# ShinYwings/SingleHDR-tf2

Measured on AMD Instinct MI355X. Metric: HDR images/sec (512x512) end-to-end inference, deq+lin+hal, higher is better.
Workload: dtype f32

## Files before the change

include/shdr.h:

```cpp
#ifndef SHDR_H_
#define SHDR_H_

#include <stdint.h>

#ifdef __cplusplus
extern "C" {
#endif

void shdr_config_reload(void);

#define SHDR_OK          0
#define SHDR_E_SHAPE    (-1)
#define SHDR_E_ALIGN    (-2)
#define SHDR_E_ARCH     (-3)
#define SHDR_E_LAUNCH   (-4)
#define SHDR_E_NULL     (-5)

#define SHDR_ACT_NONE   0
#define SHDR_ACT_RELU   1
#define SHDR_ACT_LRELU  2
#define SHDR_ACT_TANH   3

#define SHDR_ALGO_AUTO    0
#define SHDR_ALGO_MFMA    1
// ... 117 lines not shown
int shdr_invcrf_decode_fwd_f32(const float* feat, const float* wfc, const float* bfc,
                               const float* table, float* out, int B, int F, int K,
                               void* stream);
int shdr_increase_fwd_f32(const float* rf, float* out, int B, int K, void* stream);
int shdr_apply_rf_fwd_f32(const float* x, const float* rf, float* y, int B,
                          int64_t n_per_batch, int K, void* stream);

int shdr_clip_fwd_f32(const float* x, float* y, int64_t n, float lo, float hi, void* stream);
int shdr_vgg_preprocess_fwd_f32(const float* x, float* y, int64_t npix, int out_channels,
                                void* stream);
int shdr_reverse3_fwd_f32(const float* x, float* y, int64_t npix, void* stream);
int shdr_alpha_blend_fwd_f32(const float* b, const float* hal, float* a, float* alpha_out,
                             int64_t npix, float thr, void* stream);
int shdr_pack3_fwd_f32(const float* s0, const float* s1, const float* s2, const float* s3,
                       int nsrc, float* y, int out_channels, int64_t npix, void* stream);
int shdr_pad_channels_f32(const float* x, float* y, int64_t npix, int Cin, int Cout, void* stream);
int shdr_logc_fwd_f32(const float* x, float* y, int64_t n, void* stream);
int shdr_affine_act_f32(const float* x, const float* scale, const float* shift, const float* residual, float* y,
                        int64_t npix, int C, int act, void* stream);

int shdr_act_bwd_f32(const float* dy, const float* y, float* dx, int64_t n, int act, void* stream);
int shdr_clip_bwd_f32(const float* dy, const float* x, float* dx, int64_t n, float lo, float hi, void* stream);
int shdr_add_f32(const float* a, const float* b, float* y, int64_t n, void* stream);
int shdr_add_ranged_f32(const float* a, const float* b, float* y, int64_t n, float* y_range, void* stream);
int shdr_avgpool2_bwd_f32(const float* dy, float* dx, int N, int H, int W, int C, void* stream);
int shdr_maxpool2_bwd_f32(const float* x, const float* dy, float* dx, int N, int H, int W, int C, void* stream);
int shdr_maxpool3s2_bwd_f32(const float* x, const float* y, const float* dy, float* dx, int N, int H, int W, int C, void* stream);
int shdr_resize2x_bwd_f32(const float* dy, float* dx, int N, int H, int W, int C, void* stream);
int shdr_resize2x_bwd_ranged_f32(const float* dy, float* dx, int N, int H, int W, int C, float* dx_range, void* stream);
int shdr_gap_bwd_f32(const float* dy, float* dx, int N, int HW, int C, void* stream);
// ... 346 lines not shown
```

singlehdr-tf2_amd/_lib.py:

```python
import ctypes
import os

_HERE = os.path.dirname(os.path.abspath(__file__))
LIB_PATH = os.environ.get("SHDR_LIB") or os.path.join(_HERE, "libshdr.so")

c_int = ctypes.c_int
c_i64 = ctypes.c_int64
c_f32 = ctypes.c_float
c_ptr = ctypes.c_void_p


class ConvDesc(ctypes.Structure):
    _fields_ = [("N", ctypes.c_int32), ("H", ctypes.c_int32), ("W", ctypes.c_int32),
                ("C1", ctypes.c_int32), ("C2", ctypes.c_int32),
                ("Cout", ctypes.c_int32), ("KH", ctypes.c_int32), ("KW", ctypes.c_int32),
                ("stride", ctypes.c_int32), ("pad_t", ctypes.c_int32), ("pad_l", ctypes.c_int32),
                ("Ho", ctypes.c_int32), ("Wo", ctypes.c_int32),
                ("x2_scale", ctypes.c_float),
                ("act1", ctypes.c_int32), ("act2", ctypes.c_int32),
                ("res_cstride", ctypes.c_int32), ("y_cstride", ctypes.c_int32),
                ("algo", ctypes.c_int32), ("cout_valid", ctypes.c_int32),
                ("w_batch_stride", ctypes.c_int64),
                ("y_pix_stride", ctypes.c_int32), ("y_off_h", ctypes.c_int32), ("y_off_w", ctypes.c_int32),
                ("y_H", ctypes.c_int32), ("y_W", ctypes.c_int32),
# ... 101 lines not shown
    "shdr_soft_hist_fwd_f32": (c_int, [c_ptr, c_ptr, c_i64, c_int, c_int, c_ptr]),
    "shdr_lin_frontend_fwd_f32": (c_int, [c_ptr, c_ptr, c_int, c_int, c_int, c_int, c_ptr]),
    "shdr_avgpool2_fwd_f32": (c_int, [c_ptr, c_ptr, c_int, c_int, c_int, c_int, c_ptr]),
    "shdr_maxpool2_fwd_f32": (c_int, [c_ptr, c_ptr, c_int, c_int, c_int, c_int, c_ptr]),
    "shdr_maxpool3s2_fwd_f32": (c_int, [c_ptr, c_ptr, c_int, c_int, c_int, c_int, c_ptr]),
    "shdr_resize2x_fwd_f32": (c_int, [c_ptr, c_ptr, c_int, c_int, c_int, c_int, c_ptr]),
    "shdr_gap_fwd_f32": (c_int, [c_ptr, c_ptr, c_int, c_int, c_int, c_ptr]),
    "shdr_invcrf_decode_fwd_f32": (c_int, [c_ptr] * 5 + [c_int, c_int, c_int, c_ptr]),
    "shdr_increase_fwd_f32": (c_int, [c_ptr, c_ptr, c_int, c_int, c_ptr]),
    "shdr_apply_rf_fwd_f32": (c_int, [c_ptr, c_ptr, c_ptr, c_int, c_i64, c_int, c_ptr]),
    "shdr_clip_fwd_f32": (c_int, [c_ptr, c_ptr, c_i64, c_f32, c_f32, c_ptr]),
    "shdr_vgg_preprocess_fwd_f32": (c_int, [c_ptr, c_ptr, c_i64, c_int, c_ptr]),
    "shdr_reverse3_fwd_f32": (c_int, [c_ptr, c_ptr, c_i64, c_ptr]),
    "shdr_alpha_blend_fwd_f32": (c_int, [c_ptr, c_ptr, c_ptr, c_ptr, c_i64, c_f32, c_ptr]),
    "shdr_pack3_fwd_f32": (c_int, [c_ptr] * 4 + [c_int, c_ptr, c_int, c_i64, c_ptr]),
    "shdr_logc_fwd_f32": (c_int, [c_ptr, c_ptr, c_i64, c_ptr]),
    "shdr_affine_act_f32": (c_int, [c_ptr] * 5 + [c_i64, c_int, c_int, c_ptr]),
    "shdr_pad_channels_f32": (c_int, [c_ptr, c_ptr, c_i64, c_int, c_int, c_ptr]),
    "shdr_act_bwd_f32": (c_int, [c_ptr, c_ptr, c_ptr, c_i64, c_int, c_ptr]),
    "shdr_clip_bwd_f32": (c_int, [c_ptr, c_ptr, c_ptr, c_i64, c_f32, c_f32, c_ptr]),
    "shdr_add_f32": (c_int, [c_ptr, c_ptr, c_ptr, c_i64, c_ptr]),
    "shdr_add_ranged_f32": (c_int, [c_ptr, c_ptr, c_ptr, c_i64, c_ptr, c_ptr]),
    "shdr_avgpool2_bwd_f32": (c_int, [c_ptr, c_ptr, c_int, c_int, c_int, c_int, c_ptr]),
    "shdr_maxpool2_bwd_f32": (c_int, [c_ptr, c_ptr, c_ptr, c_int, c_int, c_int, c_int, c_ptr]),
    "shdr_maxpool3s2_bwd_f32": (c_int, [c_ptr, c_ptr, c_ptr, c_ptr, c_int, c_int, c_int, c_int, c_ptr]),
    "shdr_resize2x_bwd_f32": (c_int, [c_ptr, c_ptr, c_int, c_int, c_int, c_int, c_ptr]),
    "shdr_resize2x_bwd_ranged_f32": (c_int, [c_ptr, c_ptr, c_int, c_int, c_int, c_int, c_ptr, c_ptr]),
    "shdr_gap_bwd_f32": (c_int, [c_ptr, c_ptr, c_int, c_int, c_int, c_ptr]),
    "shdr_upsample_zero2_f32": (c_int, [c_ptr, c_ptr, c_int, c_int, c_int, c_int, c_ptr]),
    "shdr_bn_stats_f32": (c_int, [c_ptr] * 6 + [c_i64, c_int, c_f32, c_ptr]),
# ... 99 lines not shown
```

singlehdr-tf2_amd/_ops.py:

```python
import collections
import ctypes
import math

import numpy as np
import torch

try:
    from . import _lib
except ImportError:
    import _lib

AUTOGRAD = None


def _needs_grad(*tensors):
    return AUTOGRAD is not None and torch.is_grad_enabled() and any(
        isinstance(t, torch.Tensor) and t.requires_grad for t in tensors)


WINOGRAD = True


ACT_NONE, ACT_RELU, ACT_LRELU, ACT_TANH = 0, 1, 2, 3
ALGO_AUTO, ALGO_MFMA, ALGO_DIRECT, ALGO_MFMA_REG = 0, 1, 2, 3
# ... 740 lines not shown
        return AUTOGRAD.pack3(list(srcs), out_channels, dtype)
    lib = _lib.load()
    srcs_in = list(srcs)
    srcs = [_pix3(s, "src%d" % i)[0] for i, s in enumerate(srcs)]
    n = len(srcs)
    if not 1 <= n <= 4:
        raise ValueError("pack3: 1..4 sources")
    if any(s.shape != srcs[0].shape for s in srcs):
        raise ValueError("pack3: shape mismatch")
    oc = out_channels or 3 * n
    y = torch.empty(tuple(srcs[0].shape[:-1]) + (oc,), device=srcs[0].device, dtype=dtype)
    p = [_ptr(s) for s in srcs] + [None] * (4 - n)
    if dtype == HALF:
        _lib.check(lib.shdr_pack3_f16(p[0], p[1], p[2], p[3], n, _ptr(y), oc, srcs[0].numel() // 3, 0, _stream()), "shdr_pack3_f16")
        return y
    _lib.check(lib.shdr_pack3_fwd_f32(p[0], p[1], p[2], p[3], n, _ptr(y), oc, srcs[0].numel() // 3,
                                      _stream()), "shdr_pack3_fwd_f32")
    if n == 1:
        return _carry_range(y, srcs_in[0])
    bounds = [_bound_of(t) for t in srcs_in]
    return y if None in bounds else set_bound(y, max(bounds))


def _conv_desc(x_shape, w_shape, stride, c2, x2_scale, cout_valid):
    n, h, wd, c1 = x_shape
    kh, kw, cin, cout_gemm = w_shape
    ho, pt = same_pad(h, kh, stride)
    wo, pl = same_pad(wd, kw, stride)
    d = _lib.ConvDesc()
    d.N, d.H, d.W, d.C1, d.C2 = n, h, wd, c1, c2
    d.Cout, d.KH, d.KW, d.stride = cout_gemm, kh, kw, stride
    d.cout_valid = cout_valid or cout_gemm
    d.pad_t, d.pad_l, d.Ho, d.Wo = pt, pl, ho, wo
    d.x2_scale = float(x2_scale)
    return d

# ... 1411 lines not shown
```

singlehdr-tf2_amd/build.py:

```python
import os
import shutil
import subprocess
import sys

HERE = os.path.dirname(os.path.abspath(__file__))
CSRC = os.path.join(HERE, "csrc")
INCLUDE = os.path.normpath(os.path.join(HERE, "..", "include"))
OBJ_DIR = os.path.join(HERE, "build")
LIB = os.path.join(HERE, "libshdr.so")

SOURCES = {
    "api.cpp": [],
    "conv.hip": [],
    "conv_plan.hip": [],
    "conv_x3.hip": [],
    "conv_x3n.hip": [],
    "conv_f16.hip": [],
    "conv_f16_patch.hip": [],
    "conv_f16_w3.hip": [],
    "wgrad_x3.hip": [],
    "wgrad_f16.hip": [],
    "wgrad_f16_alltaps.hip": [],
    "elem_f16.hip": ["-ffp-contract=off"],
    "wgrad.hip": [],
    "wgrad_winograd.hip": [],
    "bwd.hip": [],
    "finetune.hip": [],
    "winograd.hip": [],
    "winograd_fused.hip": [],
    "frontend.hip": ["-ffp-contract=off"],
    "pool.hip": [],
    "up2_lowres.hip": [],
    "up2_fused.hip": [],
    "crf.hip": [],
    "glue.hip": [],
    "imageio.hip": [],
    "hdr_rle.hip": [],
    "metrics.hip": [],
    "camera.hip": ["-ffp-contract=off"],
    "dataset.hip": ["-ffp-contract=off"],
    "exr.hip": ["-ffp-contract=off"],
    "exr_write.hip": ["-ffp-contract=off"],
    "deflate.hip": [],
    "deflate_lz.hip": [],
    "inflate.hip": [],
    "hdr_real.hip": ["-ffp-contract=off"],
    "jpeg.hip": ["-ffp-contract=off"],
    "jpeg_scan.hip": [],
}
COMMON = ["-O3", "-std=c++17", "-fPIC", "--offload-arch=gfx950", "-I" + INCLUDE, "-I" + CSRC,
# ... 8 lines not shown


def _stale(target, deps):
    if not os.path.exists(target):
        return True
    t = os.path.getmtime(target)
    return any(os.path.getmtime(d) > t for d in deps)


def build(force=False, verbose=True):
    hipcc = _hipcc()
    os.makedirs(OBJ_DIR, exist_ok=True)
    headers = [os.path.join(CSRC, "shdr_internal.h"), os.path.join(CSRC, "linear_resize.h"), os.path.join(CSRC, "jpeg_int.h"), os.path.join(CSRC, "deflate_huffman.h"),
               os.path.join(CSRC, "deflate_lz.h"), os.path.join(CSRC, "deflate_batch.h"),
               os.path.join(CSRC, "inflate.h"), os.path.join(CSRC, "jpeg_scan.h"),
               os.path.join(CSRC, "exr_half.h"), os.path.join(INCLUDE, "shdr.h"), __file__]
    objs = []
    procs = []
    for src, extra in SOURCES.items():
        s = os.path.join(CSRC, src)
        o = os.path.join(OBJ_DIR, os.path.splitext(src)[0] + ".o")
        objs.append(o)
        if force or _stale(o, [s] + headers):
            cmd = [hipcc] + COMMON + extra + ["-x", "hip", "-c", s, "-o", o]
            if verbose:
                print(" ".join(cmd), flush=True)
            procs.append((src, subprocess.Popen(cmd)))
    for src, p in procs:
        if p.wait() != 0:
            raise RuntimeError("hipcc failed on " + src)
    if force or procs or _stale(LIB, objs):
# ... 10 lines not shown
```

singlehdr-tf2_amd/csrc/up2_fused.hip:

```cpp
#include <hip/hip_fp16.h>
#include <stdlib.h>

#include <type_traits>

#include "shdr_internal.h"

namespace {

using f32x4 = __attribute__((ext_vector_type(4))) float;
using f16x8 = __attribute__((ext_vector_type(8))) _Float16;

inline hipStream_t S(void* s) { return reinterpret_cast<hipStream_t>(s); }

constexpr int UF_HEADER_FLOATS = 16;
constexpr int UF_IMG_HALVES = 64 * 32, UF_UNIT_HALVES = 2 * UF_IMG_HALVES;
constexpr int UF_R = 8;
constexpr int UF_COLS = 14;
constexpr int UF_MAX_CIN = 128;
constexpr int UF_THREADS = 256;
constexpr int uf_stride(int CMAX) { return CMAX == 32 ? 32 : CMAX + 8; }

struct UpFusedArgs {
  const float* x;
  const _Float16* wp;
  const float* hdr;
  const float* bias;
  const float* scale;
  const float* shift;
  const float* proj;
  float* y;
  float* yproj;
  const unsigned* xr;
  unsigned* yr;
  int N, h, w, C1, nty, ntx, act1, act2;
  int npatch;
};

__device__ __forceinline__ void uf_range_scale(const unsigned* r, float& xs, float& ixs) {
  xs = 1.0f;
  ixs = 1.0f;
  const unsigned b = r ? *r : 0u;
  if (b != 0u && b < 0x7f800000u) {
    int ex;
    frexpf(__uint_as_float(b), &ex);
    int T = 11 - ex;
    T = T < -126 ? -126 : (T > 126 ? 126 : T);
    xs = ldexpf(1.0f, T);
    ixs = ldexpf(1.0f, -T);
  }
}
// ... 35 lines not shown
  for (int e = 0; e < 4; ++e) r[e] = __int_as_float(__builtin_amdgcn_update_dpp(0, __float_as_int(a[e]), 0x111, 0xf, 0xf, true));
  return r;
}
__device__ __forceinline__ f32x4 from_right(f32x4 a) {
  f32x4 r;
#pragma unroll
  for (int e = 0; e < 4; ++e) r[e] = __int_as_float(__builtin_amdgcn_update_dpp(0, __float_as_int(a[e]), 0x101, 0xf, 0xf, true));
  return r;
}

__device__ __forceinline__ int uf_xcd_remap(int bid, int nwg) {
  const int q = nwg >> 3, r = nwg & 7, xcd = bid & 7, idx = bid >> 3;
  return (xcd < r ? xcd * (q + 1) : r * (q + 1) + (xcd - r) * q) + idx;
}

template <int R, int CW, int CMAX>
__global__ __launch_bounds__(UF_THREADS, 2) void up2_fused_kernel(const UpFusedArgs a) {
  constexpr int UF_STRIDE = uf_stride(CMAX);
  constexpr int COUT = 16 * CW, PPB = 4 / CW, GT = 64 * CW;
  constexpr int NPIX = 16 * R, IMG = NPIX * UF_STRIDE;
  constexpr int RO = R - 2;
  extern __shared__ __attribute__((aligned(16))) _Float16 fsm_all[];

  const int lane = threadIdx.x & 63;
  const int wave = __builtin_amdgcn_readfirstlane(threadIdx.x >> 6);
  const int ps = PPB == 1 ? 0 : wave / CW;
  const int cw = PPB == 1 ? wave : wave % CW;
  const int tid = PPB == 1 ? threadIdx.x : threadIdx.x & (GT - 1);
  _Float16* const fsm = fsm_all + ps * (2 * IMG);
  const float* const projp = CW == 4 ? a.proj : nullptr;
  int L = uf_xcd_remap(blockIdx.x, gridDim.x) * PPB + ps;
// ... 180 lines not shown
          ym = fmaxf(fmaxf(fmaxf(fmaxf(ym, fabsf(v[0])), fabsf(v[1])), fabsf(v[2])), fabsf(v[3]));
        }
        if (projp) {
#pragma unroll
          for (int j = 0; j < 3; ++j) {
            float t = v[0] * pq[j][0] + v[1] * pq[j][1] + v[2] * pq[j][2] + v[3] * pq[j][3];
            t += __shfl_xor(t, 16, 64);
            t += __shfl_xor(t, 32, 64);
            if (fg == 0) part[(cw * RO * 64 + (qo * 2 + r) * 32 + 2 * p + s) * 3 + j] = t;
          }
        }
      }
  }
  if (projp) {
    __syncthreads();
    for (int slot = tid; slot < RO * 64; slot += UF_THREADS) {
      const int s = slot & 1, pp = (slot >> 1) & 15, r = (slot >> 5) & 1, qo = slot >> 6;
      const int m0 = m_start + qo, jj = j_start - 1 + pp;
      if (m0 < a.h && pp >= 1 && pp <= UF_COLS && jj < a.w) {
        float* o = a.yproj + (((size_t)n * 2 * a.h + 2 * m0 + r) * 2 * a.w + 2 * jj + s) * 3;
#pragma unroll
        for (int j = 0; j < 3; ++j)
          o[j] = ((part[slot * 3 + j] + part[(RO * 64 + slot) * 3 + j]) + part[(2 * RO * 64 + slot) * 3 + j]) + part[(3 * RO * 64 + slot) * 3 + j];
      }
    }
  }
  if (a.y && a.yr) shdr::range_out_block256(a.yr, ym);
}

constexpr int uf_lds_bytes(int R, int CW, int CMAX) { return (4 / CW) * 2 * 16 * R * uf_stride(CMAX) * 2; }

bool uf_geometry_ok(const shdr_conv2d_desc* d) {
  return d && d->N > 0 && d->H > 0 && d->W > 0 && d->H % 2 == 0 && d->W % 2 == 0 && d->KH == 3 && d->KW == 3 && d->stride == 1 && d->pad_t == 1 &&
         d->pad_l == 1 && d->Ho == d->H && d->Wo == d->W && d->C2 == 0 && d->C1 % 32 == 0 && d->C1 <= UF_MAX_CIN;
}
bool uf_shape_ok(const shdr_conv2d_desc* d) { return uf_geometry_ok(d) && d->C1 >= 64 && d->Cout == 64; }
bool uf_narrow_shape_ok(const shdr_conv2d_desc* d) {
  return uf_geometry_ok(d) && d->C1 >= 32 && (d->Cout == 32 || (d->Cout == 16 && d->C1 <= 64));
// ... 5 lines not shown
  g->N = d->N; g->H = d->H / 2; g->W = d->W / 2; g->C1 = d->C1; g->C2 = 0;
  g->Cout = uf_narrow_columns(d->Cout);
  g->KH = 1; g->KW = 1; g->stride = 1; g->pad_t = 0; g->pad_l = 0; g->Ho = g->H; g->Wo = g->W;
  g->x2_scale = 1.0f; g->act1 = SHDR_ACT_NONE; g->act2 = SHDR_ACT_NONE; g->algo = SHDR_ALGO_AUTO; g->cout_valid = g->Cout; g->y_cstride = g->Cout;
  return true;
}
__global__ __launch_bounds__(256) void up2_fused_filter_kernel(const float* __restrict__ w, float* __restrict__ st, int Cin, int Cout, int Cp) {
  const long total = (long)Cin * Cp;
  for (long e = (long)blockIdx.x * 256 + threadIdx.x; e < total; e += (long)gridDim.x * 256) {
    const int col = (int)(e % Cp), ci = (int)(e / Cp);
    const int t = col / Cout, co = col - t * Cout;
    st[e] = t < 9 ? w[((size_t)t * Cin + ci) * Cout + co] : 0.0f;
  }
}

template <int CW, int CMAX>
int uf_launch(const UpFusedArgs& a, hipStream_t st) {
  constexpr int lds = uf_lds_bytes(UF_R, CW, CMAX), PPB = 4 / CW;
  static_assert(lds <= 160 * 1024 - 64, "the patch images of a block must fit the CU's LDS");
  static bool attr_done[shdr::kMaxDevices] = {};
  const int dev_slot = shdr::device_slot();
  if (!attr_done[dev_slot]) {
    hipError_t e = hipFuncSetAttribute(reinterpret_cast<const void*>(&up2_fused_kernel<UF_R, CW, CMAX>), hipFuncAttributeMaxDynamicSharedMemorySize, lds);
    if (e != hipSuccess) return shdr::fail(SHDR_E_ARCH, "hipFuncSetAttribute: %s", hipGetErrorString(e));
    attr_done[dev_slot] = true;
  }
  const long nblk = ((long)a.npatch + PPB - 1) / PPB;
  hipLaunchKernelGGL((up2_fused_kernel<UF_R, CW, CMAX>), dim3((unsigned)nblk), dim3(UF_THREADS), lds, st, a);
  return shdr::check_launch("up2_fused_kernel");
}

}

extern "C" int shdr_conv2d_up2_narrow_enabled(void) { return SHDR_ENV("SHDR_NO_UP2_NARROW") == nullptr ? 1 : 0; }

extern "C" int shdr_conv2d_up2_fused_ok_f32(const shdr_conv2d_desc* d) {
  const bool narrow = uf_narrow_shape_ok(d) && shdr_conv2d_up2_narrow_enabled();
  if (!(uf_shape_ok(d) || narrow) || SHDR_ENV("SHDR_NO_UP2_FUSED") != nullptr || SHDR_ENV("SHDR_NO_UP2_LOWRES") != nullptr ||
      SHDR_ENV("SHDR_NO_WINOGRAD") != nullptr || SHDR_ENV("SHDR_NO_X3") != nullptr)
    return 0;
  if (d->algo != SHDR_ALGO_AUTO || d->prologue != SHDR_PROLOGUE_BILINEAR2X) return 0;
  if ((d->cout_valid != 0 && d->cout_valid != d->Cout) || d->w_batch_stride != 0 || d->y_pix_stride > 1 || (d->y_cstride != 0 && d->y_cstride != d->Cout)) return 0;
  if (d->act1 == SHDR_ACT_TANH || d->act2 == SHDR_ACT_TANH) return 0;
// ... 11 lines not shown
extern "C" int shdr_conv2d_up2_fused_prepare_filter_f32(const shdr_conv2d_desc* d, const float* w, float* prepared, void* stream) {
  if (uf_shape_ok(d)) return shdr_conv2d_up2_lowres_prepare_filter_f32(d, w, prepared, stream);
  SHDR_REQUIRE(d && w && prepared, SHDR_E_NULL, "up2_fused_prepare_filter: null pointer");
  shdr_conv2d_desc g;
  SHDR_REQUIRE(uf_narrow_gemm_desc(d, &g), SHDR_E_SHAPE,
               "up2_fused_prepare_filter: need a 3x3 layer with one source, even H and W, and Cin 64 / 96 / 128 -> 64, Cin 32 .. 128 -> 32 or Cin 32 / 64 -> 16");
  const int64_t packed = shdr_conv2d_x3_filter_elems_f32(&g);
  SHDR_REQUIRE(packed > 0, SHDR_E_SHAPE, "up2_fused_prepare_filter: the 1x1 form of this layer has no packed filter");
  float* staged = prepared + packed;
  const long total = (long)g.C1 * g.Cout;
  hipLaunchKernelGGL(up2_fused_filter_kernel, dim3(shdr::stream_grid(total)), dim3(256), 0, S(stream), w, staged, g.C1, d->Cout, g.Cout);
  if (int rc = shdr::check_launch("up2_fused_filter")) return rc;
  return shdr_conv2d_x3_prepare_filter_f32(&g, staged, prepared, stream);
}

extern "C" int shdr_conv2d_fwd_up2_fused_f32(const shdr_conv2d_desc* d, const float* x, const float* prepared, const float* bias, const float* scale,
                                             const float* shift, const float* proj, float* y_proj, float* y, const float* x_range, float* y_range,
                                             void* stream) {
  SHDR_REQUIRE(d && x && prepared && x_range, SHDR_E_NULL, "conv2d_up2_fused: null desc / x / prepared filter / x_range");
  SHDR_REQUIRE(y || y_proj, SHDR_E_NULL, "conv2d_up2_fused: neither y nor y_proj");
  SHDR_REQUIRE((proj == nullptr) == (y_proj == nullptr), SHDR_E_NULL, "conv2d_up2_fused: proj and y_proj come together");
  SHDR_REQUIRE(shdr_conv2d_up2_fused_ok_f32(d), SHDR_E_SHAPE, "conv2d_up2_fused: layer not taken (shdr_conv2d_up2_fused_ok_f32)");
  SHDR_REQUIRE(!proj || d->Cout == 64, SHDR_E_SHAPE, "conv2d_up2_fused: the projected output is the 64-cout form's");
  SHDR_REQUIRE((scale == nullptr) == (shift == nullptr), SHDR_E_NULL, "conv2d_up2_fused: scale and shift come together");
  SHDR_REQUIRE(shdr::aligned16(x) && shdr::aligned16(prepared) && (!y || shdr::aligned16(y)) && (!bias || shdr::aligned16(bias)) &&
                   (!scale || (shdr::aligned16(scale) && shdr::aligned16(shift))) && (!proj || shdr::aligned16(proj)),
               SHDR_E_ALIGN, "conv2d_up2_fused: tensors must be 16-byte aligned");
  UpFusedArgs a{};
  a.x = x; a.hdr = prepared; a.wp = reinterpret_cast<const _Float16*>(prepared + UF_HEADER_FLOATS);
  a.bias = bias; a.scale = scale; a.shift = shift; a.proj = proj; a.y = y; a.yproj = y_proj;
  a.xr = reinterpret_cast<const unsigned*>(x_range); a.yr = reinterpret_cast<unsigned*>(y_range);
  a.N = d->N; a.h = d->H / 2; a.w = d->W / 2; a.C1 = d->C1; a.act1 = d->act1; a.act2 = d->act2;
  a.nty = (a.h + UF_R - 3) / (UF_R - 2);
  a.ntx = (a.w + UF_COLS - 1) / UF_COLS;
  a.npatch = (int)((long)a.N * a.nty * a.ntx);
  hipStream_t st = S(stream);
  if (d->Cout == 64) return uf_launch<4, 128>(a, st);
  if (d->Cout == 32) return d->C1 <= 64 ? uf_launch<2, 64>(a, st) : uf_launch<2, 128>(a, st);
  return d->C1 <= 32 ? uf_launch<1, 32>(a, st) : uf_launch<1, 64>(a, st);
}
```

singlehdr-tf2_amd/hallucination_net.py:

```python
import torch

try:
    from . import _ops as K
    from ._layers import Layer, Conv2D, BatchNormalization, is_training, taping
except ImportError:
    import _ops as K
    from _layers import Layer, Conv2D, BatchNormalization, is_training, taping


class down1(Layer):

    def __init__(self, inChannels, outChannels, device=None):
        super().__init__()
        self.conv1 = Conv2D(inChannels, outChannels, (3, 3), device=device)
        self.conv2 = Conv2D(outChannels, outChannels, (3, 3), device=device)

    def call(self, x, proj=None):
        if x.shape[-1] != self.conv1.kernel.shape[2]:
            x = self.conv1.call_padded(x, cin_pad=x.shape[-1], act1=K.ACT_RELU)
        else:
            x = self.conv1(x, act1=K.ACT_RELU)
        if proj is not None:
            r = K.conv2d_maxpool2(x, self.conv2.kernel, self.conv2.bias, act1=K.ACT_RELU, proj=proj)
            if r is not None:
# ... 27 lines not shown
        self.norm1 = BatchNormalization(outChannels, device=device)

    def call(self, x, training="training"):
        if is_training(training):
            return self.norm1.train_apply(self.conv1(K.resize2x(x), act1=K.ACT_RELU), relu=True)
        if taping(x, self.conv1.kernel, self.norm1.gamma):
            return self.norm1.frozen_apply(self.conv1(K.resize2x(x), act1=K.ACT_RELU), relu=True)
        scale, shift = self.norm1.folded()
        if x.dtype != torch.float32 or not K.WINOGRAD:
            return self.conv1.call_up2(x, act1=K.ACT_RELU, scale=scale, shift=shift, act2=K.ACT_RELU)
        return self.conv1.call_up2(x, act1=K.ACT_RELU, scale=scale, shift=shift, act2=K.ACT_RELU, lowres=True)

    def call_projected(self, x, proj):
        scale, shift = self.norm1.folded()
        return self.conv1.call_up2(x, act1=K.ACT_RELU, scale=scale, shift=shift, act2=K.ACT_RELU, proj=proj, lowres=True)


class skipLayer(Layer):

    def __init__(self, xChannels, skChannels, outChannels, device=None):
        super().__init__()
        self.conv1 = Conv2D(xChannels + skChannels, outChannels, (1, 1), device=device)

    def call(self, x, sk, **kw):
        return self.conv1(x, x2=sk, x2_scale=1.0 / 255, **kw)


class model(Layer):
    def __init__(self, VGG_MEAN=(103.939, 116.779, 123.68), padding="SAME", device=None):
        super().__init__()
# ... 7 lines not shown
        self.norm1 = BatchNormalization(512, device=device)
        self.u5 = up(512, 512, device=device)
        self.s5 = skipLayer(512, 512, 512, device=device)
        self.u4 = up(512, 512, device=device)
        self.s4 = skipLayer(512, 512, 512, device=device)
        self.u3 = up(512, 256, device=device)
        self.s3 = skipLayer(256, 256, 256, device=device)
        self.u2 = up(256, 128, device=device)
        self.s2 = skipLayer(128, 128, 128, device=device)
        self.u1 = up(128, 64, device=device)
        self.s1 = skipLayer(64, 64, 64, device=device)
        self.conv2 = Conv2D(64, 3, (1, 1), device=device)
        self.norm2 = BatchNormalization(3, device=device)
        self.s0 = skipLayer(3, 3, 3, device=device)

    def call(self, input_layer, training="training"):
        train = is_training(training)
        if list(self.VGG_MEAN) != [103.939, 116.779, 123.68]:
            raise NotImplementedError("custom VGG_MEAN is not supported by the HIP preprocess kernel")
        input_layer, il = K.fork(input_layer)
        bgr = K.vgg_preprocess(input_layer)
        tail, d1_projected = None, False
        if K.native_fp16() and (train or not taping(input_layer, self.conv1.kernel, self.norm1.gamma)):
            x, d1 = self.d1(K.vgg_preprocess(il, 16, K.HALF))
        else:
            if not train and K.PRECISION == "fp32" and not taping(input_layer, self.conv1.kernel, self.norm1.gamma):
                tail = self._tail_projection()
            if tail is not None:
                x, d1, d1_projected = self.d1(K.vgg_preprocess(il, 4), proj=tail["skip_map"])
            else:
                x, d1 = self.d1(K.vgg_preprocess(il, 4))
        x, d2 = self.d2(x)
        x, d3 = self.d3(x)
        x, d4 = self.d4(x)
        enc, d5 = self.d5(x)
        enc = K.mark(enc, getattr(self, "_decoder_grads_done", None))
        frozen = not train and taping(input_layer, self.conv1.kernel, self.norm1.gamma)
        if train:
            x = self.norm1.train_apply(self.conv1(enc), relu=True)
        elif frozen:
            x = self.norm1.frozen_apply(self.conv1(enc), relu=True)
        else:
            sc, sh = self.norm1.folded()
            x = self.conv1(enc, scale=sc, shift=sh, act2=K.ACT_RELU)
        x = self.s5(self.u5(x, training), d5)
        x = self.s4(self.u4(x, training), d4)
        x = self.s3(self.u3(x, training), d3)
        x = self.s2(self.u2(x, training), d2)
        if train or frozen:
            x = self.s1(self.u1(x, training), d1)
            if train:
                x = self.norm2.train_apply(self.conv2.call_padded(x, cout_pad=16), relu=True)
            else:
                x = self.norm2.frozen_apply(self.conv2.call_padded(x, cout_pad=16), relu=True)
        else:
            sc, sh = self.norm2.folded()
            if d1_projected:
                pu = self.u1.call_projected(x, tail["up_map"])
                if pu is not None:
                    x = K.affine_act(pu, shift=tail["const"], residual=d1, act=K.ACT_RELU)
                else:
                    x = K.conv2d(self.u1(x, training), tail["up_filter"], tail["bias"], cout_valid=3, scale=sc, shift=sh, residual=d1,
                                 act2=K.ACT_RELU)
            else:
                wc, bc = self._tail_filter(d1.shape[-1])
                x = K.conv2d(self.u1(x, training), wc, bc, x2=d1, cout_valid=3, scale=sc, shift=sh, act2=K.ACT_RELU)
        return self.s0(x, bgr, act1=K.ACT_RELU)

    def _tail_projection(self):
        c_skip = self.s1.conv1.kernel.shape[2] - 64
        if c_skip != 64:
            return None
        wc, bc = self._tail_filter(c_skip)
# ... 27 lines not shown
```

singlehdr-tf2_amd/pipeline.py:

```python
import math

import torch

try:
    from . import _ops as K
    from . import metrics, tf_utils
except ImportError:
    import _ops as K
    import metrics
    import tf_utils

THRESHOLD = 0.12


PRECISIONS = ("fp32", "fp16")


class Inference:

    def __init__(self, deq, lin, hal, ref=None, threshold=THRESHOLD, streams=1, precision="fp32"):
        if precision not in PRECISIONS:
            raise ValueError("precision must be one of %s, got %r" % (PRECISIONS, precision))
        self._deq, self._lin, self._hal, self._ref = deq, lin, hal, ref
        self.threshold = threshold
# ... 14 lines not shown
            for st in self._streams:
                main.wait_stream(st)
            for o in outs:
                o.record_stream(main)
            return torch.cat(outs, dim=0)

    def _run(self, ldr, return_intermediates):
        with K.range_scope():
            return self._run_scoped(ldr, return_intermediates)

    def _run_scoped(self, ldr, return_intermediates):
        pred_deq = self._deq(ldr, training=False)
        C_pred = K.clip(pred_deq, 0.0, 1.0)
        with K.precision("fp32"):
            pred_invcrf = self._lin(C_pred, training=False)
        B_pred = tf_utils.apply_rf(C_pred, pred_invcrf)
        bgr_hal_res = self._hal(B_pred, training=False)
        A_pred = K.alpha_blend(B_pred, bgr_hal_res, self.threshold)
        out = A_pred
        if self._ref is not None and K.native_fp16():
            out = self._ref(K.pack3([A_pred, B_pred, C_pred], 16, K.HALF), training=False)
        elif self._ref is not None:
            out = self._ref(K.pack3([A_pred, B_pred, C_pred], 12), training=False)
        if return_intermediates:
            return dict(C_pred=C_pred, invcrf=pred_invcrf, B_pred=B_pred, hal=bgr_hal_res, A_pred=A_pred,
                        hdr=out if self._ref is not None else None)
        return out


class GraphedInference:

    def __init__(self, deq, lin, hal, ref=None, threshold=THRESHOLD, copy_output=False, precision="fp32"):
        self._copy_output = copy_output
# ... 360 lines not shown
```

Before: 935.5.

## Fuse inverse-CRF apply with VGG preprocess and hallucination tail with alpha blend

Adds a kernel that applies the inverse response curve and also writes the BGR and 4-channel VGG-preprocessed tensors with their abs-max range in one pass. The hallucination net's 1x1 tail convolutions, skip add and alpha blend are folded into a per-pixel epilogue, either inside the fused upsample conv kernel (new TAIL template) or as a standalone kernel. A ranged pack3 variant computes the output range during packing. The aim is to cut several small elementwise launches and intermediate memory round trips at 512x512. The cost is a new code path with extra template instantiations and register pressure in the conv kernel, plus rounding that may differ slightly from the unfused path.

After: 939.9, median of 4. No clear change (+0.5%).

```diff
diff --git a/include/shdr.h b/include/shdr.h
--- a/include/shdr.h
+++ b/include/shdr.h
@@ -155,6 +155,19 @@
                              int64_t npix, float thr, void* stream);
 int shdr_pack3_fwd_f32(const float* s0, const float* s1, const float* s2, const float* s3,
                        int nsrc, float* y, int out_channels, int64_t npix, void* stream);
+int shdr_pack3_ranged_f32(const float* s0, const float* s1, const float* s2, const float* s3,
+                          int nsrc, float* y, int out_channels, int64_t npix, float* y_range, void* stream);
+
+int shdr_glue_fuse_enabled(void);
+int shdr_rf_preprocess_f32(const float* x, const float* rf, float* b_pred, float* bgr, float* x4, float* x4_range, int B,
+                           int64_t n_per_batch, int K, void* stream);
+int shdr_hal_tail_f32(const float* yproj, const float* res, const float* konst, const float* w, float x2_scale, const float* bias,
+                      const float* bgr, const float* b_pred, float* a_pred, float* hal_out, int64_t npix, float thr, void* stream);
+int shdr_conv2d_fwd_up2_fused_tail_f32(const shdr_conv2d_desc* d, const float* x, const float* prepared, const float* bias,
+                                       const float* scale, const float* shift, const float* proj, const float* x_range, const float* res,
+                                       const float* konst, const float* w, float x2_scale, const float* tail_bias, const float* bgr,
+                                       const float* b_pred, float* a_pred, float* hal_out, float thr, void* stream);
+
 int shdr_pad_channels_f32(const float* x, float* y, int64_t npix, int Cin, int Cout, void* stream);
 int shdr_logc_fwd_f32(const float* x, float* y, int64_t n, void* stream);
 int shdr_affine_act_f32(const float* x, const float* scale, const float* shift, const float* residual, float* y,
diff --git a/singlehdr-tf2_amd/_lib.py b/singlehdr-tf2_amd/_lib.py
--- a/singlehdr-tf2_amd/_lib.py
+++ b/singlehdr-tf2_amd/_lib.py
@@ -139,6 +139,11 @@
     "shdr_reverse3_fwd_f32": (c_int, [c_ptr, c_ptr, c_i64, c_ptr]),
     "shdr_alpha_blend_fwd_f32": (c_int, [c_ptr, c_ptr, c_ptr, c_ptr, c_i64, c_f32, c_ptr]),
     "shdr_pack3_fwd_f32": (c_int, [c_ptr] * 4 + [c_int, c_ptr, c_int, c_i64, c_ptr]),
+    "shdr_pack3_ranged_f32": (c_int, [c_ptr] * 4 + [c_int, c_ptr, c_int, c_i64, c_ptr, c_ptr]),
+    "shdr_glue_fuse_enabled": (c_int, []),
+    "shdr_rf_preprocess_f32": (c_int, [c_ptr] * 6 + [c_int, c_i64, c_int, c_ptr]),
+    "shdr_hal_tail_f32": (c_int, [c_ptr] * 4 + [c_f32] + [c_ptr] * 5 + [c_i64, c_f32, c_ptr]),
+    "shdr_conv2d_fwd_up2_fused_tail_f32": (c_int, [ctypes.POINTER(ConvDesc)] + [c_ptr] * 10 + [c_f32] + [c_ptr] * 5 + [c_f32, c_ptr]),
     "shdr_logc_fwd_f32": (c_int, [c_ptr, c_ptr, c_i64, c_ptr]),
     "shdr_affine_act_f32": (c_int, [c_ptr] * 5 + [c_i64, c_int, c_int, c_ptr]),
     "shdr_pad_channels_f32": (c_int, [c_ptr, c_ptr, c_i64, c_int, c_int, c_ptr]),
diff --git a/singlehdr-tf2_amd/_ops.py b/singlehdr-tf2_amd/_ops.py
--- a/singlehdr-tf2_amd/_ops.py
+++ b/singlehdr-tf2_amd/_ops.py
@@ -778,12 +778,90 @@
     if dtype == HALF:
         _lib.check(lib.shdr_pack3_f16(p[0], p[1], p[2], p[3], n, _ptr(y), oc, srcs[0].numel() // 3, 0, _stream()), "shdr_pack3_f16")
         return y
+    bounds = [_bound_of(t) for t in srcs_in]
+    if n > 1 and None in bounds and glue_fused():
+        yr = _new_slot(y.device)
+        _lib.check(lib.shdr_pack3_ranged_f32(p[0], p[1], p[2], p[3], n, _ptr(y), oc, srcs[0].numel() // 3, _ptr(yr), _stream()),
+                   "shdr_pack3_ranged_f32")
+        return _set_range(y, yr)
     _lib.check(lib.shdr_pack3_fwd_f32(p[0], p[1], p[2], p[3], n, _ptr(y), oc, srcs[0].numel() // 3,
                                       _stream()), "shdr_pack3_fwd_f32")
     if n == 1:
         return _carry_range(y, srcs_in[0])
-    bounds = [_bound_of(t) for t in srcs_in]
     return y if None in bounds else set_bound(y, max(bounds))
+
+
+def glue_fuse_enabled():
+    return bool(_lib.load().shdr_glue_fuse_enabled())
+
+
+def glue_fused(*tensors):
+    return PRECISION == "fp32" and WINOGRAD and not EXACT_FP32 and not _needs_grad(*tensors) and glue_fuse_enabled()
+
+
+def rf_preprocess(x, rf):
+    lib = _lib.load()
+    x, _ = _pix3(x, "x")
+    rf = _chk(_d(rf), "rf")
+    b = x.shape[0]
+    if rf.shape[0] != b:
+        raise ValueError("rf_preprocess: batch mismatch %d vs %d" % (b, rf.shape[0]))
+    bp, bgr = torch.empty_like(x), torch.empty_like(x)
+    x4 = torch.empty(tuple(x.shape[:-1]) + (4,), device=x.device, dtype=torch.float32)
+    xr = _new_slot(x.device)
+    _lib.check(lib.shdr_rf_preprocess_f32(_ptr(x), _ptr(rf), _ptr(bp), _ptr(bgr), _ptr(x4), _ptr(xr), b, x.numel() // b, rf.shape[1],
+                                          _stream()), "shdr_rf_preprocess_f32")
+    return bp, bgr, _set_range(x4, xr)
+
+
+def _hal_tail_operands(npix, residual, const, w, bias, bgr, b_pred):
+    ts = [_pix3(t, nm) for t, nm in ((residual, "residual"), (bgr, "bgr"), (b_pred, "b_pred"))]
+    if any(n != npix for _, n in ts):
+        raise ValueError("hal_tail: residual, bgr and b_pred must have the pixel count of the projected output")
+    w = _chk(_d(w), "w")
+    if tuple(w.shape) != (1, 1, 6, 3) or _chk(_d(const), "const").numel() != 3 or _chk(_d(bias), "bias").numel() != 3:
+        raise ValueError("hal_tail: need a [1,1,6,3] filter, const [3] and bias [3]")
+    return ts[0][0], _d(const), w, _d(bias), ts[1][0], ts[2][0]
+
+
+def hal_tail(yproj, residual, const, w, x2_scale, bias, bgr, b_pred, thr=0.12, want_hal=False):
+    lib = _lib.load()
+    yproj, npix = _pix3(yproj, "yproj")
+    res, const, w, bias, bgr, b_pred = _hal_tail_operands(npix, residual, const, w, bias, bgr, b_pred)
+    a = torch.empty_like(yproj)
+    hal = torch.empty_like(yproj) if want_hal else None
+    _lib.check(lib.shdr_hal_tail_f32(_ptr(yproj), _ptr(res), _ptr(const), _ptr(w), float(x2_scale), _ptr(bias), _ptr(bgr), _ptr(b_pred),
+                                     _ptr(a), _ptr(hal), npix, float(thr), _stream()), "shdr_hal_tail_f32")
+    return hal, a
+
+
+def conv2d_up2_hal_tail(x, w, bias, act1, scale, shift, act2, proj, residual, const, w_tail, x2_scale, bias_tail, bgr, b_pred, thr=0.12,
+                        want_hal=False):
+    if _is_h(x) or _d(w).shape[-1] != 64:
+        return None
+    layer = _up2_layer("fused", x, w, bias, act1, scale, shift, act2)
+    if layer is None:
+        return None
+    lib = _lib.load()
+    x_in = x
+    d, x, prepared = layer
+    proj = _chk(_d(proj), "proj")
+    if tuple(proj.shape) != (3, d.Cout):
+        raise ValueError("conv2d_up2_hal_tail: proj must be [3, %d]" % d.Cout)
+    res, const, w_tail, bias_tail, bgr, b_pred = _hal_tail_operands(d.N * d.H * d.W, residual, const, w_tail, bias_tail, bgr, b_pred)
+    xr = _range_of(x_in)
+    if xr is None:
+        RANGE_MISSES[(tuple(x.shape), None, tuple(_d(w).shape))] += 1
+        xr = _new_slot(x.device)
+        _lib.check(lib.shdr_absmax_f32(_ptr(x), x.numel(), _ptr(xr), _stream()), "shdr_absmax_f32")
+    a = torch.empty((d.N, d.H, d.W, 3), device=x.device, dtype=torch.float32)
+    hal = torch.empty_like(a) if want_hal else None
+    rc = lib.shdr_conv2d_fwd_up2_fused_tail_f32(ctypes.byref(d), _ptr(x), _ptr(prepared), _ptr(_d(bias)), _ptr(_d(scale)), _ptr(_d(shift)),
+                                                _ptr(proj), _ptr(xr), _ptr(res), _ptr(const), _ptr(w_tail), float(x2_scale), _ptr(bias_tail),
+                                                _ptr(bgr), _ptr(b_pred), _ptr(a), _ptr(hal), float(thr), _stream())
+    _lib.check(rc, "shdr_conv2d_fwd_up2_fused_tail_f32")
+    PROJECTED_LAUNCHES[0] += 1
+    return hal, a
 
 
 def _conv_desc(x_shape, w_shape, stride, c2, x2_scale, cout_valid):
diff --git a/singlehdr-tf2_amd/build.py b/singlehdr-tf2_amd/build.py
--- a/singlehdr-tf2_amd/build.py
+++ b/singlehdr-tf2_amd/build.py
@@ -34,6 +34,7 @@
     "up2_fused.hip": [],
     "crf.hip": [],
     "glue.hip": [],
+    "glue_fuse.hip": [],
     "imageio.hip": [],
     "hdr_rle.hip": [],
     "metrics.hip": [],
@@ -72,7 +73,7 @@
     headers = [os.path.join(CSRC, "shdr_internal.h"), os.path.join(CSRC, "linear_resize.h"), os.path.join(CSRC, "jpeg_int.h"), os.path.join(CSRC, "deflate_huffman.h"),
                os.path.join(CSRC, "deflate_lz.h"), os.path.join(CSRC, "deflate_batch.h"),
                os.path.join(CSRC, "inflate.h"), os.path.join(CSRC, "jpeg_scan.h"),
-               os.path.join(CSRC, "exr_half.h"), os.path.join(INCLUDE, "shdr.h"), __file__]
+               os.path.join(CSRC, "exr_half.h"), os.path.join(CSRC, "hal_tail.h"), os.path.join(INCLUDE, "shdr.h"), __file__]
     objs = []
     procs = []
     for src, extra in SOURCES.items():
diff --git a/singlehdr-tf2_amd/csrc/glue_fuse.hip b/singlehdr-tf2_amd/csrc/glue_fuse.hip
--- /dev/null
+++ b/singlehdr-tf2_amd/csrc/glue_fuse.hip
@@ -0,0 +1,117 @@
+#include "hal_tail.h"
+#include "shdr_internal.h"
+
+namespace {
+
+inline hipStream_t S(void* s) { return reinterpret_cast<hipStream_t>(s); }
+
+constexpr float kVggMean0 = 103.939f, kVggMean1 = 116.779f, kVggMean2 = 123.68f;
+
+__global__ __launch_bounds__(256) void rf_preprocess_kernel(const float* __restrict__ x, const float* __restrict__ rf, float* __restrict__ bp,
+                                                            float* __restrict__ bgr, float* __restrict__ x4, unsigned* __restrict__ x4r,
+                                                            long npix_per_batch, int K) {
+  extern __shared__ float lut[];
+  const int b = blockIdx.y;
+  for (int k = threadIdx.x; k < K; k += 256) lut[k] = rf[(long)b * K + k];
+  __syncthreads();
+  const float km1 = (float)(K - 1);
+  auto one = [&](float xv) {
+#pragma clang fp contract(off)
+    const float yv = km1 * xv;
+    const float y0 = floorf(yv);
+    const float y1 = y0 + 1.0f;
+    const int i0 = min(max((int)y0, 0), K - 1);
+    const int i1 = min(max((int)y1, 0), K - 1);
+    return (y1 - yv) * lut[i0] + (yv - y0) * lut[i1];
+  };
+  const long base = (long)b * npix_per_batch;
+  float m = 0.0f;
+  for (long q = (long)blockIdx.x * 256 + threadIdx.x; q < npix_per_batch; q += (long)gridDim.x * 256) {
+    const long p = base + q;
+    const float r = one(x[3 * p]), g = one(x[3 * p + 1]), bl = one(x[3 * p + 2]);
+    bp[3 * p] = r; bp[3 * p + 1] = g; bp[3 * p + 2] = bl;
+    const float v0 = __builtin_fmaf(bl, 255.0f, -kVggMean0), v1 = __builtin_fmaf(g, 255.0f, -kVggMean1), v2 = __builtin_fmaf(r, 255.0f, -kVggMean2);
+    bgr[3 * p] = v0; bgr[3 * p + 1] = v1; bgr[3 * p + 2] = v2;
+    *reinterpret_cast<float4*>(x4 + 4 * p) = make_float4(v0, v1, v2, 0.0f);
+    m = fmaxf(fmaxf(m, fabsf(v0)), fmaxf(fabsf(v1), fabsf(v2)));
+  }
+  if (x4r) shdr::range_out_block256(x4r, m);
+}
+
+struct HalTailKernelArgs {
+  shdr::HalTailArgs t;
+  const float* yproj;
+  long npix;
+};
+
+__global__ __launch_bounds__(256) void hal_tail_kernel(const HalTailKernelArgs a) {
+  shdr::HalTailConsts c;
+  shdr::hal_tail_consts(a.t, c);
+  for (long p = (long)blockIdx.x * 256 + threadIdx.x; p < a.npix; p += (long)gridDim.x * 256) {
+    const float u[3] = {a.yproj[3 * p], a.yproj[3 * p + 1], a.yproj[3 * p + 2]};
+    shdr::hal_tail_pixel(a.t, c, (size_t)p, u);
+  }
+}
+
+struct Pack3Args { const float* s[4]; };
+
+__global__ __launch_bounds__(256) void pack3_ranged_kernel(Pack3Args src, int nsrc, float* __restrict__ y, int OC, long npix,
+                                                           unsigned* __restrict__ yr) {
+  const long total = npix * OC;
+  float m = 0.0f;
+  for (long e = (long)blockIdx.x * 256 + threadIdx.x; e < total; e += (long)gridDim.x * 256) {
+    const long p = e / OC;
+    const int ch = (int)(e - p * OC);
+    const int s = ch / 3, c = ch - 3 * s;
+    float v = 0.f;
+    if (s < nsrc) {
+      const float* sp = s == 0 ? src.s[0] : (s == 1 ? src.s[1] : (s == 2 ? src.s[2] : src.s[3]));
+      v = sp[3 * p + c];
+    }
+    y[e] = v;
+    m = fmaxf(m, fabsf(v));
+  }
+  shdr::range_out_block256(yr, m);
+}
+
+}
+
+extern "C" int shdr_glue_fuse_enabled(void) { return SHDR_ENV("SHDR_NO_GLUE_FUSE") == nullptr ? 1 : 0; }
+
+extern "C" int shdr_rf_preprocess_f32(const float* x, const float* rf, float* b_pred, float* bgr, float* x4, float* x4_range, int B,
+                                      int64_t n_per_batch, int K, void* stream) {
+  SHDR_REQUIRE(x && rf && b_pred && bgr && x4, SHDR_E_NULL, "rf_preprocess: null pointer");
+  SHDR_REQUIRE(B > 0 && B <= 65535 && n_per_batch > 0 && n_per_batch % 3 == 0 && K >= 2 && K <= 16384, SHDR_E_SHAPE,
+               "rf_preprocess: bad shape (B=%d, K=%d; n_per_batch must be a multiple of 3)", B, K);
+  SHDR_REQUIRE(shdr::aligned16(x4), SHDR_E_ALIGN, "rf_preprocess: x4 not 16-byte aligned");
+  const long npix = (long)(n_per_batch / 3);
+  int gx = shdr::stream_grid(npix);
+  if (gx > 1024) gx = 1024;
+  hipLaunchKernelGGL(rf_preprocess_kernel, dim3(gx, B), dim3(256), (size_t)K * sizeof(float), S(stream), x, rf, b_pred, bgr, x4,
+                     reinterpret_cast<unsigned*>(x4_range), npix, K);
+  return shdr::check_launch("rf_preprocess");
+}
+
+extern "C" int shdr_hal_tail_f32(const float* yproj, const float* res, const float* konst, const float* w, float x2_scale, const float* bias,
+                                 const float* bgr, const float* b_pred, float* a_pred, float* hal_out, int64_t npix, float thr, void* stream) {
+  SHDR_REQUIRE(yproj && res && konst && w && bias && bgr && b_pred && a_pred, SHDR_E_NULL, "hal_tail: null pointer");
+  SHDR_REQUIRE(npix > 0 && thr > 0.f, SHDR_E_SHAPE, "hal_tail: npix and thr must be positive");
+  HalTailKernelArgs a{};
+  a.t.res = res; a.t.konst = konst; a.t.w = w; a.t.bias = bias; a.t.bgr = bgr; a.t.bpred = b_pred; a.t.a = a_pred; a.t.hal = hal_out;
+  a.t.x2_scale = x2_scale; a.t.thr = thr; a.yproj = yproj; a.npix = (long)npix;
+  hipLaunchKernelGGL(hal_tail_kernel, dim3(shdr::stream_grid(npix)), dim3(256), 0, S(stream), a);
+  return shdr::check_launch("hal_tail");
+}
+
+extern "C" int shdr_pack3_ranged_f32(const float* s0, const float* s1, const float* s2, const float* s3, int nsrc, float* y, int out_channels,
+                                     int64_t npix, float* y_range, void* stream) {
+  SHDR_REQUIRE(y && s0 && y_range, SHDR_E_NULL, "pack3_ranged: null pointer");
+  SHDR_REQUIRE(nsrc >= 1 && nsrc <= 4 && out_channels >= 3 * nsrc && npix > 0, SHDR_E_SHAPE,
+               "pack3_ranged: need 1<=nsrc<=4, out_channels>=3*nsrc");
+  const float* s[4] = {s0, s1, s2, s3};
+  for (int i = 0; i < nsrc; ++i) SHDR_REQUIRE(s[i], SHDR_E_NULL, "pack3_ranged: source %d is null", i);
+  Pack3Args pa{{s0, s1, s2, s3}};
+  hipLaunchKernelGGL(pack3_ranged_kernel, dim3(shdr::stream_grid(npix * out_channels)), dim3(256), 0, S(stream), pa, nsrc, y, out_channels,
+                     (long)npix, reinterpret_cast<unsigned*>(y_range));
+  return shdr::check_launch("pack3_ranged");
+}
diff --git a/singlehdr-tf2_amd/csrc/hal_tail.h b/singlehdr-tf2_amd/csrc/hal_tail.h
--- /dev/null
+++ b/singlehdr-tf2_amd/csrc/hal_tail.h
@@ -0,0 +1,54 @@
+#pragma once
+#include "shdr_internal.h"
+
+namespace shdr {
+
+struct HalTailArgs {
+  const float* res;
+  const float* konst;
+  const float* w;
+  const float* bias;
+  const float* bgr;
+  const float* bpred;
+  float* a;
+  float* hal;
+  float x2_scale, thr;
+};
+
+struct HalTailConsts {
+  float w[6][3], k[3], b[3];
+};
+__device__ __forceinline__ void hal_tail_consts(const HalTailArgs& a, HalTailConsts& c) {
+#pragma clang fp contract(off)
+#pragma unroll
+  for (int i = 0; i < 6; ++i)
+#pragma unroll
+    for (int n = 0; n < 3; ++n) c.w[i][n] = i >= 3 ? __fmul_rn(a.w[i * 3 + n], a.x2_scale) : a.w[i * 3 + n];
+#pragma unroll
+  for (int n = 0; n < 3; ++n) { c.k[n] = a.konst[n]; c.b[n] = a.bias[n]; }
+}
+
+__device__ __forceinline__ void hal_tail_pixel(const HalTailArgs& a, const HalTailConsts& c, size_t p, const float (&u)[3]) {
+#pragma clang fp contract(off)
+  float t[6], h[3];
+#pragma unroll
+  for (int i = 0; i < 3; ++i) t[i] = fmaxf(__fadd_rn(__fadd_rn(u[i], c.k[i]), a.res[3 * p + i]), 0.0f);
+#pragma unroll
+  for (int i = 0; i < 3; ++i) t[3 + i] = __fmul_rn(a.bgr[3 * p + i], 1.0f);
+#pragma unroll
+  for (int n = 0; n < 3; ++n) {
+    float acc = 0.0f;
+#pragma unroll
+    for (int i = 0; i < 6; ++i) acc = __builtin_fmaf(t[i], c.w[i][n], acc);
+    h[n] = fmaxf(__fadd_rn(acc, c.b[n]), 0.0f);
+  }
+  if (a.hal) { a.hal[3 * p] = h[0]; a.hal[3 * p + 1] = h[1]; a.hal[3 * p + 2] = h[2]; }
+  const float b0 = a.bpred[3 * p], b1 = a.bpred[3 * p + 1], b2 = a.bpred[3 * p + 2];
+  const float mx = fmaxf(fmaxf(b0, b1), b2);
+  const float al = fminf(1.0f, __fdiv_rn(fmaxf(0.0f, __fadd_rn(__fadd_rn(mx, -1.0f), a.thr)), a.thr));
+  a.a[3 * p] = __builtin_fmaf(al, h[2], b0);
+  a.a[3 * p + 1] = __builtin_fmaf(al, h[1], b1);
+  a.a[3 * p + 2] = __builtin_fmaf(al, h[0], b2);
+}
+
+}
diff --git a/singlehdr-tf2_amd/csrc/up2_fused.hip b/singlehdr-tf2_amd/csrc/up2_fused.hip
--- a/singlehdr-tf2_amd/csrc/up2_fused.hip
+++ b/singlehdr-tf2_amd/csrc/up2_fused.hip
@@ -3,6 +3,7 @@
 
 #include <type_traits>
 
+#include "hal_tail.h"
 #include "shdr_internal.h"
 
 namespace {
@@ -34,6 +35,7 @@
   unsigned* yr;
   int N, h, w, C1, nty, ntx, act1, act2;
   int npatch;
+  shdr::HalTailArgs tail;
 };
 
 __device__ __forceinline__ void uf_range_scale(const unsigned* r, float& xs, float& ixs) {
@@ -99,7 +101,7 @@
   return (xcd < r ? xcd * (q + 1) : r * (q + 1) + (xcd - r) * q) + idx;
 }
 
-template <int R, int CW, int CMAX>
+template <int R, int CW, int CMAX, bool TAIL = false>
 __global__ __launch_bounds__(UF_THREADS, 2) void up2_fused_kernel(const UpFusedArgs a) {
   constexpr int UF_STRIDE = uf_stride(CMAX);
   constexpr int COUT = 16 * CW, PPB = 4 / CW, GT = 64 * CW;
@@ -310,14 +312,24 @@
   }
   if (projp) {
     __syncthreads();
+    shdr::HalTailConsts tc;
+    if constexpr (TAIL) shdr::hal_tail_consts(a.tail, tc);
     for (int slot = tid; slot < RO * 64; slot += UF_THREADS) {
       const int s = slot & 1, pp = (slot >> 1) & 15, r = (slot >> 5) & 1, qo = slot >> 6;
       const int m0 = m_start + qo, jj = j_start - 1 + pp;
       if (m0 < a.h && pp >= 1 && pp <= UF_COLS && jj < a.w) {
-        float* o = a.yproj + (((size_t)n * 2 * a.h + 2 * m0 + r) * 2 * a.w + 2 * jj + s) * 3;
+        const size_t pix = ((size_t)n * 2 * a.h + 2 * m0 + r) * 2 * a.w + 2 * jj + s;
+        float u[3];
 #pragma unroll
         for (int j = 0; j < 3; ++j)
-          o[j] = ((part[slot * 3 + j] + part[(RO * 64 + slot) * 3 + j]) + part[(2 * RO * 64 + slot) * 3 + j]) + part[(3 * RO * 64 + slot) * 3 + j];
+          u[j] = ((part[slot * 3 + j] + part[(RO * 64 + slot) * 3 + j]) + part[(2 * RO * 64 + slot) * 3 + j]) + part[(3 * RO * 64 + slot) * 3 + j];
+        if constexpr (TAIL) {
+          shdr::hal_tail_pixel(a.tail, tc, pix, u);
+        } else {
+          float* o = a.yproj + pix * 3;
+#pragma unroll
+          for (int j = 0; j < 3; ++j) o[j] = u[j];
+        }
       }
     }
   }
@@ -353,19 +365,19 @@
   }
 }
 
-template <int CW, int CMAX>
+template <int CW, int CMAX, bool TAIL = false>
 int uf_launch(const UpFusedArgs& a, hipStream_t st) {
   constexpr int lds = uf_lds_bytes(UF_R, CW, CMAX), PPB = 4 / CW;
   static_assert(lds <= 160 * 1024 - 64, "the patch images of a block must fit the CU's LDS");
   static bool attr_done[shdr::kMaxDevices] = {};
   const int dev_slot = shdr::device_slot();
   if (!attr_done[dev_slot]) {
-    hipError_t e = hipFuncSetAttribute(reinterpret_cast<const void*>(&up2_fused_kernel<UF_R, CW, CMAX>), hipFuncAttributeMaxDynamicSharedMemorySize, lds);
+    hipError_t e = hipFuncSetAttribute(reinterpret_cast<const void*>(&up2_fused_kernel<UF_R, CW, CMAX, TAIL>), hipFuncAttributeMaxDynamicSharedMemorySize, lds);
     if (e != hipSuccess) return shdr::fail(SHDR_E_ARCH, "hipFuncSetAttribute: %s", hipGetErrorString(e));
     attr_done[dev_slot] = true;
   }
   const long nblk = ((long)a.npatch + PPB - 1) / PPB;
-  hipLaunchKernelGGL((up2_fused_kernel<UF_R, CW, CMAX>), dim3((unsigned)nblk), dim3(UF_THREADS), lds, st, a);
+  hipLaunchKernelGGL((up2_fused_kernel<UF_R, CW, CMAX, TAIL>), dim3((unsigned)nblk), dim3(UF_THREADS), lds, st, a);
   return shdr::check_launch("up2_fused_kernel");
 }
 
@@ -407,12 +419,12 @@
   return shdr_conv2d_x3_prepare_filter_f32(&g, staged, prepared, stream);
 }
 
-extern "C" int shdr_conv2d_fwd_up2_fused_f32(const shdr_conv2d_desc* d, const float* x, const float* prepared, const float* bias, const float* scale,
-                                             const float* shift, const float* proj, float* y_proj, float* y, const float* x_range, float* y_range,
-                                             void* stream) {
+static int up2_fused_run(const shdr_conv2d_desc* d, const float* x, const float* prepared, const float* bias, const float* scale,
+                         const float* shift, const float* proj, float* y_proj, float* y, const float* x_range, float* y_range,
+                         const shdr::HalTailArgs* tail, void* stream) {
   SHDR_REQUIRE(d && x && prepared && x_range, SHDR_E_NULL, "conv2d_up2_fused: null desc / x / prepared filter / x_range");
-  SHDR_REQUIRE(y || y_proj, SHDR_E_NULL, "conv2d_up2_fused: neither y nor y_proj");
-  SHDR_REQUIRE((proj == nullptr) == (y_proj == nullptr), SHDR_E_NULL, "conv2d_up2_fused: proj and y_proj come together");
+  SHDR_REQUIRE(y || y_proj || tail, SHDR_E_NULL, "conv2d_up2_fused: neither y nor y_proj");
+  SHDR_REQUIRE((proj == nullptr) == (y_proj == nullptr && tail == nullptr), SHDR_E_NULL, "conv2d_up2_fused: proj and y_proj come together");
   SHDR_REQUIRE(shdr_conv2d_up2_fused_ok_f32(d), SHDR_E_SHAPE, "conv2d_up2_fused: layer not taken (shdr_conv2d_up2_fused_ok_f32)");
   SHDR_REQUIRE(!proj || d->Cout == 64, SHDR_E_SHAPE, "conv2d_up2_fused: the projected output is the 64-cout form's");
   SHDR_REQUIRE((scale == nullptr) == (shift == nullptr), SHDR_E_NULL, "conv2d_up2_fused: scale and shift come together");
@@ -428,7 +440,29 @@
   a.ntx = (a.w + UF_COLS - 1) / UF_COLS;
   a.npatch = (int)((long)a.N * a.nty * a.ntx);
   hipStream_t st = S(stream);
+  if (tail) {
+    a.tail = *tail;
+    return uf_launch<4, 128, true>(a, st);
+  }
   if (d->Cout == 64) return uf_launch<4, 128>(a, st);
   if (d->Cout == 32) return d->C1 <= 64 ? uf_launch<2, 64>(a, st) : uf_launch<2, 128>(a, st);
   return d->C1 <= 32 ? uf_launch<1, 32>(a, st) : uf_launch<1, 64>(a, st);
 }
+
+extern "C" int shdr_conv2d_fwd_up2_fused_f32(const shdr_conv2d_desc* d, const float* x, const float* prepared, const float* bias, const float* scale,
+                                             const float* shift, const float* proj, float* y_proj, float* y, const float* x_range, float* y_range,
+                                             void* stream) {
+  return up2_fused_run(d, x, prepared, bias, scale, shift, proj, y_proj, y, x_range, y_range, nullptr, stream);
+}
+
+extern "C" int shdr_conv2d_fwd_up2_fused_tail_f32(const shdr_conv2d_desc* d, const float* x, const float* prepared, const float* bias,
+                                                  const float* scale, const float* shift, const float* proj, const float* x_range, const float* res,
+                                                  const float* konst, const float* w, float x2_scale, const float* tail_bias, const float* bgr,
+                                                  const float* b_pred, float* a_pred, float* hal_out, float thr, void* stream) {
+  SHDR_REQUIRE(d && proj && res && konst && w && tail_bias && bgr && b_pred && a_pred, SHDR_E_NULL, "conv2d_up2_fused_tail: null pointer");
+  SHDR_REQUIRE(d->Cout == 64 && thr > 0.f, SHDR_E_SHAPE, "conv2d_up2_fused_tail: the projected output is the 64-cout form's; thr must be positive");
+  shdr::HalTailArgs t{};
+  t.res = res; t.konst = konst; t.w = w; t.bias = tail_bias; t.bgr = bgr; t.bpred = b_pred; t.a = a_pred; t.hal = hal_out;
+  t.x2_scale = x2_scale; t.thr = thr;
+  return up2_fused_run(d, x, prepared, bias, scale, shift, proj, nullptr, nullptr, x_range, nullptr, &t, stream);
+}
diff --git a/singlehdr-tf2_amd/hallucination_net.py b/singlehdr-tf2_amd/hallucination_net.py
--- a/singlehdr-tf2_amd/hallucination_net.py
+++ b/singlehdr-tf2_amd/hallucination_net.py
@@ -65,6 +65,10 @@
     def call_projected(self, x, proj):
         scale, shift = self.norm1.folded()
         return self.conv1.call_up2(x, act1=K.ACT_RELU, scale=scale, shift=shift, act2=K.ACT_RELU, proj=proj, lowres=True)
+
+    def call_projected_tail(self, x, proj, *tail):
+        scale, shift = self.norm1.folded()
+        return K.conv2d_up2_hal_tail(x, self.conv1.kernel, self.conv1.bias, K.ACT_RELU, scale, shift, K.ACT_RELU, proj, *tail)
 
 
 class skipLayer(Layer):
@@ -102,22 +106,23 @@
         self.norm2 = BatchNormalization(3, device=device)
         self.s0 = skipLayer(3, 3, 3, device=device)
 
-    def call(self, input_layer, training="training"):
+    def call(self, input_layer, training="training", head=None, blend=None):
         train = is_training(training)
         if list(self.VGG_MEAN) != [103.939, 116.779, 123.68]:
             raise NotImplementedError("custom VGG_MEAN is not supported by the HIP preprocess kernel")
         input_layer, il = K.fork(input_layer)
-        bgr = K.vgg_preprocess(input_layer)
+        bgr = head[0] if head is not None else K.vgg_preprocess(input_layer)
         tail, d1_projected = None, False
         if K.native_fp16() and (train or not taping(input_layer, self.conv1.kernel, self.norm1.gamma)):
             x, d1 = self.d1(K.vgg_preprocess(il, 16, K.HALF))
         else:
             if not train and K.PRECISION == "fp32" and not taping(input_layer, self.conv1.kernel, self.norm1.gamma):
                 tail = self._tail_projection()
+            x4 = head[1] if head is not None else K.vgg_preprocess(il, 4)
             if tail is not None:
-                x, d1, d1_projected = self.d1(K.vgg_preprocess(il, 4), proj=tail["skip_map"])
+                x, d1, d1_projected = self.d1(x4, proj=tail["skip_map"])
             else:
-                x, d1 = self.d1(K.vgg_preprocess(il, 4))
+                x, d1 = self.d1(x4)
         x, d2 = self.d2(x)
         x, d3 = self.d3(x)
         x, d4 = self.d4(x)
@@ -144,7 +149,15 @@
         else:
             sc, sh = self.norm2.folded()
             if d1_projected:
+                s0 = self.s0.conv1
+                fuse = blend is not None and s0.bias is not None and K.glue_fused(x, d1, bgr, blend[0])
+                if fuse:
+                    r = self.u1.call_projected_tail(x, tail["up_map"], d1, tail["const"], s0.kernel, 1.0 / 255, s0.bias, bgr, *blend)
+                    if r is not None:
+                        return r
                 pu = self.u1.call_projected(x, tail["up_map"])
+                if pu is not None and fuse:
+                    return K.hal_tail(pu, d1, tail["const"], s0.kernel, 1.0 / 255, s0.bias, bgr, *blend)
                 if pu is not None:
                     x = K.affine_act(pu, shift=tail["const"], residual=d1, act=K.ACT_RELU)
                 else:
diff --git a/singlehdr-tf2_amd/pipeline.py b/singlehdr-tf2_amd/pipeline.py
--- a/singlehdr-tf2_amd/pipeline.py
+++ b/singlehdr-tf2_amd/pipeline.py
@@ -52,9 +52,14 @@
         C_pred = K.clip(pred_deq, 0.0, 1.0)
         with K.precision("fp32"):
             pred_invcrf = self._lin(C_pred, training=False)
-        B_pred = tf_utils.apply_rf(C_pred, pred_invcrf)
-        bgr_hal_res = self._hal(B_pred, training=False)
-        A_pred = K.alpha_blend(B_pred, bgr_hal_res, self.threshold)
+        if not return_intermediates and K.glue_fused(C_pred, pred_invcrf):
+            B_pred, bgr, x4 = K.rf_preprocess(C_pred, pred_invcrf)
+            r = self._hal(B_pred, training=False, head=(bgr, x4), blend=(B_pred, self.threshold, False))
+            bgr_hal_res, A_pred = r if isinstance(r, tuple) else (r, K.alpha_blend(B_pred, r, self.threshold))
+        else:
+            B_pred = tf_utils.apply_rf(C_pred, pred_invcrf)
+            bgr_hal_res = self._hal(B_pred, training=False)
+            A_pred = K.alpha_blend(B_pred, bgr_hal_res, self.threshold)
         out = A_pred
         if self._ref is not None and K.native_fp16():
             out = self._ref(K.pack3([A_pred, B_pred, C_pred], 16, K.HALF), training=False)
```
